# intel/rho-diffusion

Measured on AMD Instinct MI355X. Metric: denoising_steps_per_sec, higher is better.
Workload: dtype bf16; 1 GPU; DDPM reverse step, UNetv2 3D 64^3 mc=64 (BASELINE configs[2]), batch 32/GPU, bf16, LinearSchedule(1000,1e-3,0.02); global_batch=32, hip_graph=True

## Files before the change

### rho_diffusion_amd/csrc/conv.hip

```cpp
#include <cstdio>
#include <cstdlib>
#include <type_traits>

#include "conv_common.h"

#define RHO_GB_WIDE 3
#ifndef RHO_GB_BM32
#define RHO_GB_BM32 1
#endif

struct ConvK {
    const char* x1;
    const char* x2;
    const float* pre_a;
    const float* pre_b;
    const char* w;
    const float* bias;
    const char* res;
    const float* res_add;
    char* y;
    char* y2;
    int c1, c2, cin;
    int cout, coutp, split;
    int D, H, W;
// ... 4 lines not shown
    int tiles_h, tiles_w;
    int res_add_stride;
    int y2_cl;
    const char* res2;
    int pair_lg;
    int zs_h, zs_w;
    int Hs, Ws;
    float* stats;
    int tps;
    int lgTW, lgTH;
    float inv_ihw, inv_iw;
    int cofast;
    int coef_off;
    int pad_h, pad_w, oy_mul, oy_add, ox_mul, ox_add, Ho_out, Wo_out;
    int stats_off;
    int iy_mul, iy_add, ix_mul, ix_add;
    const char* gnb_x1;
    const char* gnb_x2;
    const float* gnb_a;
    const float* gnb_b;
    int gnb_c1, gnb_silu;
    int ksplit;
    float* slab;
    long long slab_stride;
    const char* sk_x1;
    const char* sk_x2;
    const char* sk_w;
    const float* sk_bias;
    int sk_c1, sk_c2;
    const char* gna_g;
    const float* gna_cA;
    const float* gna_cP;
    const float* gna_cQ;
};

__device__ __forceinline__ int fdiv_small(int a, float inv) { return (int)(((float)a + 0.5f) * inv); }


__device__ __forceinline__ int unit_position(int u, int k, int TW, int pair_lg) {
    if (TW == 8 && pair_lg >= 0) {
        const int lo = u & ((1 << pair_lg) - 1);
        const int row = ((u >> pair_lg) << (pair_lg + 1)) | lo | ((k >> 3) << pair_lg);
        return row * 8 + (k & 7);
    }
    return u * 16 + k;
}
__device__ __forceinline__ int tile_position(int m, int c, int TW, int pair_lg) {
    const int q = c >> 2;
    const int g = (0x96 >> q) & 1;
    const int k = ((q >> 1) << 2) | (c & 3);
    return unit_position(2 * m + g, k, TW, pair_lg);
}

__device__ __forceinline__ int m16_hb(int i) { return (0x0FF0 >> i) & 1; }
__device__ __forceinline__ int m16_k8(int i) { return m16_hb(i) ? i - 4 : (i < 4 ? i : i - 8); }
__device__ __forceinline__ int tile_position16(int m16, int i, int TW, int pair_lg) {
    return unit_position(2 * (m16 >> 1) + m16_hb(i), 2 * m16_k8(i) + (m16 & 1), TW, pair_lg);
}

template <typename T, int KD, int KH, int KW, int BM, int MAXP, int NW, bool M16 = false, bool FSK = false, bool GNA = false>
__global__ __launch_bounds__(NW * 64, (NW == 8 || (KD * KH * KW == 1 && MAXP <= 10)) ? 2 : 1) void k_conv(const ConvK p) {
    extern __shared__ __attribute__((aligned(16))) char smem[];
    constexpr int CK = ET<T>::CK;
    constexpr int PE = ET<T>::PE;
    constexpr int NT = KD * KH * KW;
    constexpr int NTHR = NW * 64;
    constexpr int RPP = NTHR / 4;
    constexpr int WCO = NW / 4;
    constexpr int MT = BM / 32 / WCO;
    constexpr int WROWS = (BM + RPP - 1) / RPP;

    char* const halo = smem;
    char* const wbuf = smem + (size_t)p.NP * PITCH;

    const int tid = threadIdx.x;
    const int lane = tid & 63;
    const int wave = tid >> 6;
    const int wpos = wave & 3;
    const int wco = wave >> 2;
    const int half = lane >> 5;
    const int piece = tid & 3;

    int bt = blockIdx.x;
    int ct = blockIdx.y;
    if (p.cofast) {
        const int L = blockIdx.x + gridDim.x * blockIdx.y;
        const int slot = L >> 3;
        ct = slot % (int)gridDim.y;
        bt = (L & 7) * ((int)gridDim.x >> 3) + slot / (int)gridDim.y;
    } else {
        const int nt = gridDim.x, per = nt >> 3;
        if (per > 0) {
            const int full = per << 3;
            if (bt < full) bt = (bt & 7) * per + (bt >> 3);
        }
    }
    const int tw_i = bt % p.tiles_w;
    const int th_i = (bt / p.tiles_w) % p.tiles_h;
    const int td_i = bt / (p.tiles_w * p.tiles_h);
    const int co0 = ct * BM;
    const bool splitk = (KD != 3) && p.ksplit > 1;
    const int n = splitk ? 0 : (int)blockIdx.z;
    const int od0 = td_i * p.TD, oh0 = th_i * p.TH, ow0 = tw_i * p.TW;
    const int gd_base = od0 - (KD / 2);
    const int gh_base = p.up_h ? (oh0 / 2 - 1) : (oh0 * p.sh - p.pad_h);
    const int gw_base = p.up_w ? (ow0 / 2 - 1) : (ow0 * p.sw - p.pad_w);

    constexpr int NSMP = (KD == 3) ? 1 : MAXP;
    int spos[MAXP];
    int ssmp[NSMP];
    {
        const int ihw = p.IH * p.IW;
#pragma unroll
        for (int i = 0; i < MAXP; ++i) {
            const int hp = (tid >> 2) + RPP * i;
            int pos = -2, smp = 0;
            if (hp < p.NP) {
                const int id = fdiv_small(hp, p.inv_ihw);
                const int r = hp - id * ihw;
                const int ih = fdiv_small(r, p.inv_iw);
                const int iw = r - ih * p.IW;
                const int gd = gd_base + id;
                int gh = gh_base + ih, gw = gw_base + iw;
                bool ok = ((unsigned)gd < (unsigned)p.D) & ((unsigned)gh < (unsigned)p.H) & ((unsigned)gw < (unsigned)p.W);
                if (p.zs_h) { ok = ok && ((gh & 1) == 0) && ((gh >> 1) < p.Hs); gh >>= 1; }
                if (p.zs_w) { ok = ok && ((gw & 1) == 0) && ((gw >> 1) < p.Ws); gw >>= 1; }
                if (ok) {
                    pos = ((n * p.D + gd) * p.Hs + (gh * p.iy_mul + p.iy_add)) * p.Ws + (gw * p.ix_mul + p.ix_add);
                    if constexpr (KD != 3) smp = (int)((long long)pos / p.S_in);
                } else {
                    pos = -1;
                }
            }
            spos[i] = pos;
            if constexpr (KD != 3) ssmp[i] = smp;
        }
    }

    int offd[2], offh[2][KH], offw[2][KW];
#pragma unroll
    for (int j = 0; j < 2; ++j) {
        const int pp = M16 ? tile_position16(2 * (wpos * 2 + j), lane & 15, p.TW, p.pair_lg)
                           : tile_position(wpos * 2 + j, lane & 31, p.TW, p.pair_lg);
        const int pw = pp & (p.TW - 1);
        const int ph = (pp >> p.lgTW) & (p.TH - 1);
        const int pd = pp >> (p.lgTW + p.lgTH);
        offd[j] = pd * p.IH * p.IW * PITCH + 16 * (M16 ? (lane >> 4) : half);
#pragma unroll
        for (int kh = 0; kh < KH; ++kh) {
            const int ih = p.up_h ? (((ph + kh - 1) >> 1) + 1) : (ph * p.sh + kh);
            offh[j][kh] = ih * p.IW * PITCH;
        }
#pragma unroll
        for (int kw = 0; kw < KW; ++kw) {
            const int iw = p.up_w ? (((pw + kw - 1) >> 1) + 1) : (pw * p.sw + kw);
            offw[j][kw] = iw * PITCH;
        }
    }
    const int a_off = M16 ? (wco * (BM / WCO) + 16 * m16_hb(lane & 15) + 2 * m16_k8(lane & 15)) * PITCH + 16 * (lane >> 4)
                          : (wco * (BM / WCO) + (lane & 31)) * PITCH + 16 * half;

    f32x16_t acc[MT][2];
#pragma unroll
    for (int mi = 0; mi < MT; ++mi)
#pragma unroll
        for (int j = 0; j < 2; ++j)
#pragma unroll
            for (int r = 0; r < 16; ++r) acc[mi][j][r] = 0.0f;

    int ck_lo = 0, nck = p.cin / CK;
    if (splitk) {
        const int nall = nck, kz = (int)blockIdx.z;
        ck_lo = (int)((long long)nall * kz / p.ksplit);
        nck = (int)((long long)nall * (kz + 1) / p.ksplit) - ck_lo;
    }
    const size_t wrow_bytes = (size_t)p.cin * sizeof(T);

    const bool w_active = (BM >= RPP) || (tid < BM * 4);
    const char* const w_src0 = p.w + (size_t)co0 * wrow_bytes + (size_t)ck_lo * 64;
    unsigned w_voff = (unsigned)(tid >> 2) * (unsigned)wrow_bytes + (unsigned)piece * 16u;
    const size_t w_tap_stride = (size_t)p.coutp * wrow_bytes;
    int w_row = tid >> 2;
    if constexpr (M16) w_row = (w_row & ~31) + 16 * m16_hb(w_row & 15) + 2 * m16_k8(w_row & 15) + ((w_row >> 4) & 1);
    const int w_dst0 = w_row * PITCH + piece * 16;
    constexpr int G = 1;
    constexpr int NS = NT / G;
    constexpr int PD = (NS % 3 == 0) ? 3 : 1;
    constexpr int SLOT = G * BM * PITCH;
    uint4 wq0[PD][G], wq1[PD][G];
#pragma unroll
    for (int i = 0; i < PD; ++i)
#pragma unroll
        for (int g = 0; g < G; ++g) wq0[i][g] = wq1[i][g] = make_uint4(0u, 0u, 0u, 0u);
#define RHO_LOAD_W(set_, ck_, st_)                                                                       \
    do {                                                                                                \
        _Pragma("unroll") for (int g_ = 0; g_ < G; ++g_) {                                              \
            const char* ws_ = w_src0 + (size_t)((st_) * G + g_) * w_tap_stride + (size_t)(ck_) * 64;    \
            if (w_active) wq0[set_][g_] = *reinterpret_cast<const uint4*>(ws_ + w_voff);                \
            if constexpr (WROWS == 2) wq1[set_][g_] = *reinterpret_cast<const uint4*>(ws_ + RPP * wrow_bytes + w_voff); \
        }                                                                                               \
    } while (0)
#define RHO_LOAD_WP(set_, st_)                                                                          \
    do {                                                                                                \
        if (w_active) wq0[set_][0] = *reinterpret_cast<const uint4*>(wl + w_voff);                      \
        if constexpr (WROWS == 2) wq1[set_][0] = *reinterpret_cast<const uint4*>(wl + RPP * wrow_bytes + w_voff); \
        if (((st_) + LD) % NS == NS - 1) wl = w_src0 + (size_t)min(ck + ((st_) + LD) / NS + 1, nck - 1) * 64; \
        else wl += w_tap_stride;                                                                        \
    } while (0)
#define RHO_STORE_W(buf_, set_)                                                                         \
    do {                                                                                                \
        _Pragma("unroll") for (int g_ = 0; g_ < G; ++g_) {                                              \
            char* wd_ = wbuf + (size_t)(buf_) * SLOT + g_ * BM * PITCH + w_dst0;                        \
            if (w_active) *reinterpret_cast<uint4*>(wd_) = wq0[set_][g_];                               \
            if constexpr (WROWS == 2) *reinterpret_cast<uint4*>(wd_ + RPP * PITCH) = wq1[set_][g_];     \
        }                                                                                               \
    } while (0)

    constexpr bool PIPE = (NS % 3 == 0) && (G == 1);
    constexpr int GB = (NS % 9 == 0 && ((BM == 128 && NW == 8 && M16) || (RHO_GB_BM32 && BM == 32 && !M16))) ? RHO_GB_WIDE : 1;
    constexpr int RS = (GB == 3) ? 9 : 3;
    constexpr int DS = GB + 1;
    constexpr int LD = DS + 2;
    const float* coef = nullptr;
    if constexpr (NT != 1 && KD == 3) {
        if (p.coef_off > 0 && p.pre_a != nullptr) {
            float* cw_ = reinterpret_cast<float*>(smem + p.coef_off);
            for (int i = tid; i < p.cin; i += NTHR) {
                cw_[i] = p.pre_a[(size_t)n * p.cin + i];
                cw_[p.cin + i] = p.pre_b[(size_t)n * p.cin + i];
            }
            coef = cw_;
            __syncthreads();
        }
    }
    if constexpr (FSK) {
        static_assert(M16 && MT == 2 && KD == 3, "folded skip: the 64-couts-per-wave 16x16x32 layout of the 3-D kernels");
        typedef float f32x4_t __attribute__((ext_vector_type(4)));
        typedef unsigned int u32x4_t __attribute__((ext_vector_type(4)));
        constexpr int XR = 256 / RPP;
        const int skc = p.sk_c1 + p.sk_c2, nsk = skc / CK;
        char* const sa = smem;
        char* const sw = smem + 2 * 256 * PITCH;
        int gp[XR];
#pragma unroll
        for (int i = 0; i < XR; ++i) {
            const int r = (tid >> 2) + RPP * i;
            const int od = od0 + (r >> (p.lgTW + p.lgTH)), oh = oh0 + ((r >> p.lgTW) & (p.TH - 1)), ow = ow0 + (r & (p.TW - 1));
            const bool ok = od < p.Do && oh < p.Ho && ow < p.Wo;
            gp[i] = ok ? ((n * p.Do + od) * p.Ho + oh) * p.Wo + ow : -1;
        }
        int cb[2];
#pragma unroll
        for (int j = 0; j < 2; ++j)
            cb[j] = tile_position16(2 * (wpos * 2 + j), lane & 15, p.TW, p.pair_lg) * PITCH + 16 * (lane >> 4);
        const unsigned skw_voff = (unsigned)(tid >> 2) * (unsigned)skc * (unsigned)sizeof(T) + (unsigned)piece * 16u;
        const char* const skw0 = p.sk_w + (size_t)co0 * skc * sizeof(T);
        uint4 xr[XR], wr0 = make_uint4(0u, 0u, 0u, 0u), wr1 = make_uint4(0u, 0u, 0u, 0u);
        auto sk_load = [&](int c) {
            const int ch = c * CK;
            const char* src;
            int cs, csrc;
            if (ch < p.sk_c1) { src = p.sk_x1; cs = p.sk_c1; csrc = ch; } else { src = p.sk_x2; cs = p.sk_c2; csrc = ch - p.sk_c1; }
#pragma unroll
            for (int i = 0; i < XR; ++i) {
                const int ps = gp[i] > 0 ? gp[i] : 0;
                xr[i] = *reinterpret_cast<const uint4*>(src + ((size_t)ps * cs + csrc) * sizeof(T) + piece * 16);
            }
            const char* ws_ = skw0 + (size_t)c * 64;
            if (w_active) wr0 = *reinterpret_cast<const uint4*>(ws_ + skw_voff);
            if constexpr (WROWS == 2) wr1 = *reinterpret_cast<const uint4*>(ws_ + (size_t)RPP * skc * sizeof(T) + skw_voff);
        };
        auto sk_store = [&](int slot) {
// ... 423 lines not shown
            RHO_ONE_TAIL(0, I0, std::true_type)
            if constexpr (DX == 4) {
                RHO_ONE_TAIL(1, I1, std::true_type)
                RHO_ONE_TAIL(2, I2, std::true_type)
            }
        } else {
            int ck0 = 0;
            for (; ck0 + DX <= nck; ck0 += DX) {
                RHO_ONE_STEP(0, I0, std::false_type)
                RHO_ONE_STEP(1, I1, std::false_type)
                if constexpr (DX == 4) {
                    RHO_ONE_STEP(2, I2, std::false_type)
                    RHO_ONE_STEP(3, I3, std::false_type)
                }
            }
            RHO_ONE_TAIL(0, I0, std::false_type)
            if constexpr (DX == 4) {
                RHO_ONE_TAIL(1, I1, std::false_type)
                RHO_ONE_TAIL(2, I2, std::false_type)
            }
        }
#undef RHO_ONE_STEP
#undef RHO_ONE_TAIL
    }
#undef RHO_PHASE
#undef RHO_FENCE
#undef RHO_LOAD_W
#undef RHO_LOAD_WP
#undef RHO_STORE_W
#undef RHO_HALO_LOAD
    const __attribute__((address_space(4))) ConvK* qp = (const __attribute__((address_space(4))) ConvK*)__builtin_amdgcn_kernarg_segment_ptr();
    asm volatile("" : "+s"(qp));
    const __attribute__((address_space(4))) ConvK& q = *qp;
    if (splitk) {
        float* const slab = q.slab + (size_t)blockIdx.z * q.slab_stride;
#pragma unroll
        for (int jx = 0; jx < (M16 ? 4 : 2); ++jx) {
            const int pp = M16 ? tile_position16(wpos * 4 + jx, lane & 15, q.TW, q.pair_lg) : tile_position(wpos * 2 + jx, lane & 31, q.TW, q.pair_lg);
            const int pw = pp & (q.TW - 1);
            const int ph = (pp >> q.lgTW) & (q.TH - 1);
            const int pd = pp >> (q.lgTW + q.lgTH);
            const int od = od0 + pd, oh = oh0 + ph, ow = ow0 + pw;
            if (od >= q.Do || oh >= q.Ho || ow >= q.Wo) continue;
            const size_t L = ((size_t)od * q.Ho + oh) * q.Wo + ow;
            const int j = M16 ? (jx >> 1) : jx;
#pragma unroll
            for (int mi = 0; mi < MT; ++mi) {
#pragma unroll
                for (int rx = 0; rx < (M16 ? 2 : 4); ++rx) {
                    const int rg = M16 ? 2 * rx + (jx & 1) : rx;
                    const int co = M16 ? co0 + wco * (BM / WCO) + 16 * (2 * mi + rx) + 4 * (lane >> 4)
                                       : co0 + wco * (BM / WCO) + mi * 32 + rg * 8 + half * 4;
                    *reinterpret_cast<float4*>(slab + L * q.coutp + co) =
                        make_float4(acc[mi][j][rg * 4 + 0], acc[mi][j][rg * 4 + 1], acc[mi][j][rg * 4 + 2], acc[mi][j][rg * 4 + 3]);
                }
            }
        }
        return;
    }
    const bool reg2 = q.y2_cl && co0 >= q.split && ((q.cout - q.split) % PE == 0);
    const bool cl_region = (co0 < q.split) || reg2;
    if (cl_region) {
        const int rw = reg2 ? q.cout - q.split : q.split;
        const int rc0 = reg2 ? co0 - q.split : co0;
        char* const ry = reg2 ? q.y2 : q.y;
        const char* const rrp = reg2 ? q.res2 : q.res;
        const float* const radd = reg2 ? nullptr : q.res_add;
        constexpr int ROWB = BM * 4 + 16;
        constexpr int PPR = BM / PE;
        static_assert(NTHR % PPR == 0, "a thread keeps one channel piece across its rows (statistics accumulators)");
        char* const stg = smem;
        float ssum[PE], ssq[PE];
#pragma unroll
        for (int e = 0; e < PE; ++e) ssum[e] = ssq[e] = 0.0f;
        {
            __syncthreads();
            {
#pragma unroll
                for (int j = 0; j < 2; ++j) {
#pragma unroll
                    for (int mi = 0; mi < MT; ++mi)
#pragma unroll
                        for (int rg = 0; rg < 4; ++rg) {
                            const int lr = M16 ? wpos * 64 + (2 * j + (rg & 1)) * 16 + (lane & 15) : wpos * 64 + j * 32 + (lane & 31);
                            const int cl = M16 ? wco * (BM / WCO) + 16 * (2 * mi + (rg >> 1)) + 4 * (lane >> 4)
                                               : wco * (BM / WCO) + mi * 32 + rg * 8 + half * 4;
                            *reinterpret_cast<float4*>(stg + lr * ROWB + cl * 4) =
                                make_float4(acc[mi][j][rg * 4 + 0], acc[mi][j][rg * 4 + 1], acc[mi][j][rg * 4 + 2], acc[mi][j][rg * 4 + 3]);
                        }
                }
            }
            constexpr int NIT = 256 * PPR / NTHR;
            static_assert(256 * PPR % NTHR == 0, "whole items per thread");
            int eoff[NIT];
            uint4 rres[GNA ? 1 : NIT];
            uint4 gx[NIT];
            float bia[PE];
            float gna[PE], gnb[PE];
            const bool gnb_on = q.gnb_x1 != nullptr;
            const bool gna_on = GNA && q.gna_g != nullptr;
            uint4 gg[GNA ? NIT : 1];
            float gca[GNA ? PE : 1], gcp[GNA ? PE : 1], gcq[GNA ? PE : 1];
            {
                const int piece = tid % PPR;
                const int gco = co0 + piece * PE;
                const bool g_first = gco < q.gnb_c1;
                const char* const gsrc = g_first ? q.gnb_x1 : q.gnb_x2;
                const int gC = gna_on ? q.cout : q.split;
                const int gcs = g_first ? q.gnb_c1 : gC - q.gnb_c1, gch = g_first ? gco : gco - q.gnb_c1;
                if (gnb_on) {
                    const int nsg = n + bt / q.tps;
#pragma unroll
                    for (int e = 0; e < PE; ++e) {
                        gna[e] = q.gnb_a[(size_t)nsg * gC + gco + e];
                        gnb[e] = q.gnb_b[(size_t)nsg * gC + gco + e];
                    }
                    if constexpr (GNA) {
                        const int cpg = gC / 32;
#pragma unroll
                        for (int e = 0; e < PE; ++e) {
                            const int ce = (gco + e < gC) ? gco + e : gC - 1;
                            gca[e] = q.gna_cA[(size_t)nsg * gC + ce];
                            gcp[e] = q.gna_cP[(size_t)nsg * 32 + ce / cpg];
                            gcq[e] = q.gna_cQ[(size_t)nsg * 32 + ce / cpg];
                        }
                    }
                }
#pragma unroll
                for (int q4 = 0; q4 < PE / 4; ++q4) {
                    const float4 b4 = *reinterpret_cast<const float4*>(q.bias + co0 + piece * PE + q4 * 4);
                    bia[q4 * 4 + 0] = b4.x; bia[q4 * 4 + 1] = b4.y; bia[q4 * 4 + 2] = b4.z; bia[q4 * 4 + 3] = b4.w;
                    if constexpr (FSK) {
                        if (q.sk_bias != nullptr) {
                            const float4 s4 = *reinterpret_cast<const float4*>(q.sk_bias + co0 + piece * PE + q4 * 4);
                            bia[q4 * 4 + 0] += s4.x; bia[q4 * 4 + 1] += s4.y; bia[q4 * 4 + 2] += s4.z; bia[q4 * 4 + 3] += s4.w;
                        }
                    }
                    if constexpr (KD == 3) {
                        if (radd != nullptr) {
                            const float4 e = *reinterpret_cast<const float4*>(radd + (long long)n * q.res_add_stride + co0 + piece * PE + q4 * 4);
                            bia[q4 * 4 + 0] += e.x; bia[q4 * 4 + 1] += e.y; bia[q4 * 4 + 2] += e.z; bia[q4 * 4 + 3] += e.w;
                        }
                    }
                }
#pragma unroll
                for (int k = 0; k < NIT; ++k) {
                    const int lr = tid / PPR + k * (NTHR / PPR);
                    const int pp = M16 ? tile_position16((lr >> 6) * 4 + ((lr >> 4) & 3), lr & 15, q.TW, q.pair_lg)
                                       : tile_position((lr >> 6) * 2 + ((lr >> 5) & 1), lr & 31, q.TW, q.pair_lg);
                    const int pw = pp & (q.TW - 1);
                    const int ph = (pp >> q.lgTW) & (q.TH - 1);
                    const int pd = pp >> (q.lgTW + q.lgTH);
                    const int od = od0 + pd, oh = oh0 + ph, ow = ow0 + pw;
                    const bool ok = od < q.Do && oh < q.Ho && ow < q.Wo && (rc0 + piece * PE + PE <= rw);
                    const int L = ((n * q.Do + od) * q.Ho_out + (oh * q.oy_mul + q.oy_add)) * q.Wo_out + (ow * q.ox_mul + q.ox_add);
                    eoff[k] = ok ? L : -1;
                    if constexpr (!GNA) {
                        rres[k] = make_uint4(0u, 0u, 0u, 0u);
                        if (ok && rrp != nullptr)
                            rres[k] = *reinterpret_cast<const uint4*>(rrp + ((size_t)(unsigned)L * (unsigned)rw + (unsigned)(rc0 + piece * PE)) * sizeof(T));
                    }
                    gx[k] = make_uint4(0u, 0u, 0u, 0u);
                    if (ok && gnb_on) gx[k] = *reinterpret_cast<const uint4*>(gsrc + ((size_t)(unsigned)L * (unsigned)gcs + (unsigned)gch) * sizeof(T));
                    if constexpr (GNA) {
                        gg[k] = make_uint4(0u, 0u, 0u, 0u);
                        if (ok) gg[k] = *reinterpret_cast<const uint4*>(q.gna_g + ((size_t)(unsigned)L * (unsigned)gC + (unsigned)gco) * sizeof(T));
                    }
                }
            }
            __syncthreads();
#pragma unroll
            for (int k = 0; k < NIT; ++k) {
                if (eoff[k] < 0) continue;
                const int lr = tid / PPR + k * (NTHR / PPR), piece = tid % PPR;
                const int L = eoff[k];
                const int co = co0 + piece * PE;
                float v[PE];
#pragma unroll
                for (int q4 = 0; q4 < PE / 4; ++q4) {
                    const float4 a4 = *reinterpret_cast<const float4*>(stg + lr * ROWB + (piece * PE + q4 * 4) * 4);
                    v[q4 * 4 + 0] = a4.x + bia[q4 * 4 + 0]; v[q4 * 4 + 1] = a4.y + bia[q4 * 4 + 1];
                    v[q4 * 4 + 2] = a4.z + bia[q4 * 4 + 2]; v[q4 * 4 + 3] = a4.w + bia[q4 * 4 + 3];
                }
                if (KD != 3 && radd != nullptr) {
                    const long long ns = (long long)L / q.S_out;
#pragma unroll
                    for (int q4 = 0; q4 < PE / 4; ++q4) {
                        const float4 e = *reinterpret_cast<const float4*>(radd + ns * q.res_add_stride + co + q4 * 4);
                        v[q4 * 4 + 0] += e.x; v[q4 * 4 + 1] += e.y; v[q4 * 4 + 2] += e.z; v[q4 * 4 + 3] += e.w;
// ... 69 lines not shown
                            float dz = v[e];
                            if (q.gnb_silu) dz *= dsilu_f(fmaf(gna[e], xv[e], gnb[e]));
                            ssum[e] += dz;
                            ssq[e] = fmaf(dz, xv[e], ssq[e]);
                        }
                    } else {
#pragma unroll
                        for (int e = 0; e < PE; ++e) {
                            ssum[e] += v[e];
                            ssq[e] = fmaf(v[e], v[e], ssq[e]);
                        }
                    }
                }
            }
        }
        if (q.stats != nullptr) {
            __syncthreads();
            float* red = reinterpret_cast<float*>(stg);
#pragma unroll
            for (int e = 0; e < PE; ++e) {
                red[tid * (2 * PE) + e] = ssum[e];
                red[tid * (2 * PE) + PE + e] = ssq[e];
            }
            __syncthreads();
            const int ns = n + bt / q.tps, ts = bt % q.tps + q.stats_off;
            for (int item = tid; item < PPR * 2 * PE; item += NTHR) {
                const int piece = item / (2 * PE), e2 = item % (2 * PE);
                float accv = 0.0f;
                for (int q = 0; q < NTHR / PPR; ++q) accv += red[(q * PPR + piece) * (2 * PE) + e2];
                const int stat = e2 / PE, ch = co0 + piece * PE + (e2 % PE);
                q.stats[(((size_t)ns * q.tps + ts) * 2 + stat) * q.split + ch] = accv;
            }
        }
        return;
    }
#pragma unroll
    for (int jx = 0; jx < (M16 ? 4 : 2); ++jx) {
        const int pp = M16 ? tile_position16(wpos * 4 + jx, lane & 15, q.TW, q.pair_lg) : tile_position(wpos * 2 + jx, lane & 31, q.TW, q.pair_lg);
        const int pw = pp & (q.TW - 1);
        const int ph = (pp >> q.lgTW) & (q.TH - 1);
        const int pd = pp >> (q.lgTW + q.lgTH);
        const int od = od0 + pd, oh = oh0 + ph, ow = ow0 + pw;
        if (od >= q.Do || oh >= q.Ho || ow >= q.Wo) continue;
        const long long L = (((long long)n * q.Do + od) * q.Ho + oh) * q.Wo + ow;
        const long long ns = L / q.S_out;
        const long long ps = L - ns * q.S_out;
        const int j = M16 ? (jx >> 1) : jx;
#pragma unroll
        for (int mi = 0; mi < MT; ++mi) {
#pragma unroll
            for (int rx = 0; rx < (M16 ? 2 : 4); ++rx) {
                const int rg = M16 ? 2 * rx + (jx & 1) : rx;
                const int co = M16 ? co0 + wco * (BM / WCO) + 16 * (2 * mi + rx) + 4 * (lane >> 4)
                                   : co0 + wco * (BM / WCO) + mi * 32 + rg * 8 + half * 4;
                const float4 bv = *reinterpret_cast<const float4*>(q.bias + co);
                float v0 = acc[mi][j][rg * 4 + 0] + bv.x;
                float v1 = acc[mi][j][rg * 4 + 1] + bv.y;
                float v2 = acc[mi][j][rg * 4 + 2] + bv.z;
                float v3 = acc[mi][j][rg * 4 + 3] + bv.w;
                if (cl_region) {
                    if (q.res_add != nullptr) {
                        const float4 e = *reinterpret_cast<const float4*>(q.res_add + ns * q.res_add_stride + co);
                        v0 += e.x; v1 += e.y; v2 += e.z; v3 += e.w;
                    }
                    const size_t eo = (size_t)L * q.split + co;
                    if constexpr (sizeof(T) == 2) {
                        if (q.res != nullptr) {
                            const uint2 r = *reinterpret_cast<const uint2*>(q.res + eo * 2);
// ... 12 lines not shown
                    const int w2 = q.cout - q.split;
                    const size_t eo = (size_t)L * w2 + (co - q.split);
                    if (co < q.cout) {
                        if constexpr (sizeof(T) == 2) {
                            if (q.res2 != nullptr) {
                                const uint2 r = *reinterpret_cast<const uint2*>(q.res2 + eo * 2);
                                v0 += __uint_as_float(r.x << 16); v1 += __uint_as_float(r.x & 0xFFFF0000u);
                                v2 += __uint_as_float(r.y << 16); v3 += __uint_as_float(r.y & 0xFFFF0000u);
                            }
                            *reinterpret_cast<uint2*>(q.y2 + eo * 2) = make_uint2(pack_bf16x2(v0, v1), pack_bf16x2(v2, v3));
                        } else {
                            if (q.res2 != nullptr) {
                                const float4 r = *reinterpret_cast<const float4*>(q.res2 + eo * 4);
                                v0 += r.x; v1 += r.y; v2 += r.z; v3 += r.w;
                            }
                            *reinterpret_cast<float4*>(q.y2 + eo * 4) = make_float4(v0, v1, v2, v3);
                        }
                    }
                } else {
                    const float vv[4] = {v0, v1, v2, v3};
#pragma unroll
                    for (int e = 0; e < 4; ++e) {
                        if (co + e < q.cout) {
                            const size_t eo = ((size_t)ns * (q.cout - q.split) + (co + e - q.split)) * q.S_out + ps;
                            if (q.y2_f32 || sizeof(T) == 4)
                                reinterpret_cast<float*>(q.y2)[eo] = vv[e];
                            else
                                reinterpret_cast<bf16_raw*>(q.y2)[eo] = f32_to_bf16(vv[e]);
                        }
                    }
                }
            }
        }
    }
}

struct SplitMap {
    int Ho, Wo, Ho_out, Wo_out, oy_mul, oy_add, ox_mul, ox_add;
};
struct SplitOut {
    int cout, coutp, split;
    const float* bias;
    const float* res_add;
    long long res_add_stride, S_out;
    const char* res;
    char* y;
    const char* res2;
    char* y2;
};
template <typename T>
__global__ __launch_bounds__(256) void k_splitk_reduce(const float* __restrict__ slab, long long slab_stride, int ksplit, long long positions,
                                                       SplitOut o, SplitMap m) {
    const int c4 = o.coutp / 4;
    const long long item = (long long)blockIdx.x * 256 + threadIdx.x;
    if (item >= positions * c4) return;
    const long long Ls = item / c4;
    int co = (int)(item - Ls * c4) * 4;
    if (co >= o.cout) return;
    const size_t so = (size_t)Ls * o.coutp + co;
    float4 a = *reinterpret_cast<const float4*>(slab + so);
    for (int s = 1; s < ksplit; ++s) {
        const float4 b = *reinterpret_cast<const float4*>(slab + (size_t)s * slab_stride + so);
        a.x += b.x; a.y += b.y; a.z += b.z; a.w += b.w;
    }
    long long L = Ls;
    if (m.oy_mul != 1 || m.ox_mul != 1) {
// ... 92 lines not shown
#define RHO_CASE(bm)                                                                   \
    if (BM == bm) {                                                                    \
        if (np <= 640) return launch_one<T, KD, KH, KW, bm, 10, 4>(k, grid, lds, st);  \
        if constexpr (!PHASE) return launch_one<T, KD, KH, KW, bm, 28, 4>(k, grid, lds, st); \
    }
    RHO_CASE(32)
    RHO_CASE(64)
#undef RHO_CASE
    return RHO_E_ARG;
}

template <typename T>
int launch_taps(const rho_conv_desc& d, const ConvK& k, int BM, int np, dim3 grid, size_t lds, bool m16, hipStream_t st) {
    if (d.kd == 3 && d.kh == 3 && d.kw == 3) return launch_bm<T, 3, 3, 3>(k, BM, np, grid, lds, m16, st);
    if (d.kd == 1 && d.kh == 3 && d.kw == 3) return launch_bm<T, 1, 3, 3>(k, BM, np, grid, lds, m16, st);
    if (d.kd == 1 && d.kh == 1 && d.kw == 3) return launch_bm<T, 1, 1, 3>(k, BM, np, grid, lds, m16, st);
    if (d.kd == 1 && d.kh == 1 && d.kw == 1) return launch_bm<T, 1, 1, 1>(k, BM, np, grid, lds, m16, st);
    if (d.kd == 3 && d.kh == 2 && d.kw == 2) return launch_bm<T, 3, 2, 2>(k, BM, np, grid, lds, m16, st);
    if (d.kd == 1 && d.kh == 2 && d.kw == 2) return launch_bm<T, 1, 2, 2>(k, BM, np, grid, lds, m16, st);
    if (d.kd == 1 && d.kh == 1 && d.kw == 2) return launch_bm<T, 1, 1, 2>(k, BM, np, grid, lds, m16, st);
    if (d.kd == 3 && d.kh == 1 && d.kw == 1) return launch_bm<T, 3, 1, 1>(k, BM, np, grid, lds, m16, st);
    if (d.kd == 3 && d.kh == 1 && d.kw == 2) return launch_bm<T, 3, 1, 2>(k, BM, np, grid, lds, m16, st);
    if (d.kd == 3 && d.kh == 2 && d.kw == 1) return launch_bm<T, 3, 2, 1>(k, BM, np, grid, lds, m16, st);
    return RHO_E_ARG;
}

}

static bool m16_env_on() {
    static const bool on = !(getenv("RHO_CONV_M16") && atoi(getenv("RHO_CONV_M16")) == 0);
    return on;
}

static int conv_impl(const rho_conv_desc* dp, void* stream, int64_t* stats_tiles, int64_t* ws_want = nullptr) {
    if (!dp) return RHO_E_ARG;
    const rho_conv_desc& d = *dp;
    if (!d.x1 || !d.w || !d.bias) return RHO_E_ARG;
    if (d.dtype != RHO_F32 && d.dtype != RHO_BF16) return RHO_E_ARG;
    const int CK = d.dtype == RHO_BF16 ? 32 : 16;
    const int c2 = d.x2 ? d.c2 : 0;
    const int cin = d.c1 + c2;
    if (d.c1 <= 0 || d.c1 % CK || c2 % CK) return RHO_E_ALIGN;
    if (d.cout <= 0 || d.coutp < d.cout || d.coutp % 32 || d.split < 0 || d.split > d.cout || d.split % 32) return RHO_E_ARG;
    if (d.split > 0 && !d.y) return RHO_E_ARG;
    if (d.split < d.cout && !d.y2) return RHO_E_ARG;
    if (d.split < d.cout && d.split > 0 && d.coutp != d.cout && !d.y2_cl) return RHO_E_ARG;
    if (d.y2_cl && ((d.cout - d.split) % 4 != 0)) return RHO_E_ALIGN;
    if ((d.zs_h || d.zs_w) && (d.up_h || d.up_w || d.sh != 1 || d.sw != 1 || d.out_h <= 0 || d.out_w <= 0)) return RHO_E_ARG;
    if (d.split == d.cout && d.coutp != d.cout) return RHO_E_ARG;
    if ((d.sh != 1 && d.sh != 2) || (d.sw != 1 && d.sw != 2)) return RHO_E_ARG;
    if ((d.up_h && d.sh != 1) || (d.up_w && d.sw != 1)) return RHO_E_ARG;
    if ((d.up_h && d.kh != 3) || (d.up_w && d.kw != 3)) return RHO_E_ARG;
    if (d.n <= 0 || d.d <= 0 || d.h <= 0 || d.w_ <= 0) return RHO_E_ARG;
    if (d.ph_h < 0 || d.ph_h > 2 || d.ph_w < 0 || d.ph_w > 2) return RHO_E_ARG;
    if ((d.ph_h && ((d.kh != 2 && d.kh != 1) || d.sh != 1 || d.up_h || d.zs_h)) || (d.ph_w && ((d.kw != 2 && d.kw != 1) || d.sw != 1 || d.up_w || d.zs_w)))
        return RHO_E_ARG;
    if ((!d.ph_h && !d.phd_h && d.kh == 2) || (!d.ph_w && !d.phd_w && d.kw == 2)) return RHO_E_ARG;
    if ((d.ph_h || d.ph_w) && (d.split != d.cout || d.kd == 2)) return RHO_E_ARG;
    if (d.phd_h < 0 || d.phd_h > 2 || d.phd_w < 0 || d.phd_w > 2) return RHO_E_ARG;
    if ((d.phd_h && ((d.kh != 2 && d.kh != 1) || d.sh != 1 || d.up_h || d.zs_h || d.ph_h)) ||
        (d.phd_w && ((d.kw != 2 && d.kw != 1) || d.sw != 1 || d.up_w || d.zs_w || d.ph_w)))
        return RHO_E_ARG;
    if ((d.ph_h || d.phd_h || d.ph_w || d.phd_w) && d.kd * d.kh * d.kw == 1) return RHO_E_ARG;
    if ((d.phd_h || d.phd_w) && (d.kd == 2 || d.pre_a)) return RHO_E_ARG;

    if (conv32_applies(d)) {
        if (stats_tiles) { *stats_tiles = conv32_wps(d); return 0; }
        if (ws_want) { *ws_want = 0; return 0; }
        if (g_variant != nullptr) { snprintf(g_variant->buf, (size_t)g_variant->cap, "k_conv32<bf16>"); return 0; }
        if (d.stats && d.split != d.cout) return RHO_E_ARG;
        return launch_conv32(d, as_stream(stream));
    }

    const int hv = d.zs_h ? d.out_h : d.h, wv = d.zs_w ? d.out_w : d.w_;
    const int ho = (d.ph_h || d.phd_h) ? d.h : d.up_h ? d.h * 2 : (hv + 2 * (d.kh / 2) - d.kh) / d.sh + 1;
    const int wo = (d.ph_w || d.phd_w) ? d.w_ : d.up_w ? d.w_ * 2 : (wv + 2 * (d.kw / 2) - d.kw) / d.sw + 1;
    const int ho_out = d.ph_h ? 2 * ho : ho, wo_out = d.ph_w ? 2 * wo : wo;
    const int n_phase = (d.ph_h ? 2 : 1) * (d.ph_w ? 2 : 1);
    const int phase_idx = (d.ph_h ? d.ph_h - 1 : 0) * (d.ph_w ? 2 : 1) + (d.ph_w ? d.ph_w - 1 : 0);
    const int dout = d.d;

    ConvK k{};
    int gridz = d.n;
    k.pad_h = d.kh == 1 ? 0 : d.ph_h ? 2 - d.ph_h : d.phd_h ? d.phd_h - 1 : d.kh / 2;
    k.pad_w = d.kw == 1 ? 0 : d.ph_w ? 2 - d.ph_w : d.phd_w ? d.phd_w - 1 : d.kw / 2;
    k.iy_mul = d.phd_h ? 2 : 1; k.iy_add = d.phd_h ? d.phd_h - 1 : 0;
    k.ix_mul = d.phd_w ? 2 : 1; k.ix_add = d.phd_w ? d.phd_w - 1 : 0;
    k.oy_mul = d.ph_h ? 2 : 1; k.oy_add = d.ph_h ? d.ph_h - 1 : 0;
    k.ox_mul = d.ph_w ? 2 : 1; k.ox_add = d.ph_w ? d.ph_w - 1 : 0;
    if (d.kd == 1 && d.kh == 1 && d.kw == 1) {
        if (d.sh != 1 || d.sw != 1 || d.up_h || d.up_w) return RHO_E_ARG;
        k.D = 1; k.H = 1; k.W = d.n * d.d * d.h * d.w_;
        k.Do = 1; k.Ho = 1; k.Wo = k.W;
        gridz = 1;
    } else if (d.kd == 1) {
        k.D = d.n * d.d; k.H = hv; k.W = wv;
        k.Do = k.D; k.Ho = ho; k.Wo = wo;
        gridz = 1;
    } else {
        k.D = d.d; k.H = hv; k.W = wv;
        k.Do = dout; k.Ho = ho; k.Wo = wo;
// ... 103 lines not shown
        k.gna_g = (const char*)d.gna_g; k.gna_cA = d.gna_cA; k.gna_cP = d.gna_cP; k.gna_cQ = d.gna_cQ;
        k.tps = (int)tps_geo;
    } else if (d.gnb_x1) {
        if (!d.stats || !d.gnb_a || !d.gnb_b || d.gnb_c1 <= 0 || d.gnb_c1 > d.split || d.gnb_c1 % 32 || (d.split - d.gnb_c1) % 32 ||
            ((d.gnb_c1 < d.split) != (d.gnb_x2 != nullptr)))
            return RHO_E_ARG;
        k.gnb_x1 = (const char*)d.gnb_x1; k.gnb_x2 = (const char*)d.gnb_x2; k.gnb_a = d.gnb_a; k.gnb_b = d.gnb_b;
        k.gnb_c1 = d.gnb_c1; k.gnb_silu = d.gnb_silu;
    }
    size_t lds = (size_t)t.NP * PITCH + (size_t)WSLOTS * BM * PITCH;
    k.sk_w = nullptr;
    size_t lds_sk = 0;
    if (d.sk_w) {
        if (!d.sk_x1 || d.sk_c1 <= 0 || d.sk_c1 % CK || d.sk_c2 < 0 || d.sk_c2 % CK || ((d.sk_c2 > 0) != (d.sk_x2 != nullptr))) return RHO_E_ARG;
        if (!(m16 && m16_env_on() && d.kd == 3 && d.kh == 3 && d.kw == 3 && t.NP <= 640 && (BM == 64 || BM == 128) && d.split == d.cout &&
              !d.zs_h && !d.zs_w && !d.ph_h && !d.ph_w && !d.phd_h && !d.phd_w))
            return RHO_E_ARG;
        k.sk_x1 = (const char*)d.sk_x1; k.sk_x2 = (const char*)d.sk_x2; k.sk_w = (const char*)d.sk_w; k.sk_bias = d.sk_bias;
        k.sk_c1 = d.sk_c1; k.sk_c2 = d.sk_c2;
        lds_sk = (size_t)2 * 256 * PITCH + (size_t)2 * BM * PITCH;
    }
    k.coef_off = 0;
    if (taps > 1 && d.kd == 3 && d.pre_a && lds + (size_t)2 * cin * sizeof(float) <= (BM == 128 ? lds_cap : lds_cap / 2)) {
        k.coef_off = (int)lds;
        lds += (size_t)2 * cin * sizeof(float);
    }
    if (taps == 1)
        lds = (size_t)2 * 256 * PITCH + (size_t)2 * BM * PITCH + (d.pre_a ? (size_t)2 * k.cin * sizeof(float) : 0);
    if (k.coef_off > 0 && (size_t)k.coef_off < lds_sk) { lds -= (size_t)2 * cin * sizeof(float); k.coef_off = 0; }
    if (lds < lds_sk) lds = lds_sk;
    if (d.stats) { const size_t lr = (size_t)(BM == 128 ? 512 : 256) * 16 * sizeof(float); if (lds < lr) lds = lr; }
    const size_t lds_epi = (size_t)256 * (BM * 4 + 16);
    if ((d.split > 0 || d.y2_cl) && lds < lds_epi) lds = lds_epi;
    hipStream_t st = as_stream(stream);
    const bool m16_env = m16_env_on();
    const int rc = d.dtype == RHO_BF16 ? launch_taps<bf16_raw>(d, k, BM, t.NP, grid, lds, m16 && m16_env, st)
                                       : launch_taps<float>(d, k, BM, t.NP, grid, lds, false, st);
    if (rc != 0 || ksplit == 1 || g_variant != nullptr) return rc;
    const long long items = positions * (d.coutp / 4);
    const dim3 rgrid((unsigned)((items + 255) / 256));
    const SplitMap sm{k.Ho, k.Wo, k.Ho_out, k.Wo_out, k.oy_mul, k.oy_add, k.ox_mul, k.ox_add};
    const SplitOut so{d.cout, d.coutp, d.split, d.bias, d.res_add, (long long)k.res_add_stride, k.S_out, (const char*)d.res, (char*)d.y,
                      (const char*)d.res2, (char*)d.y2};
    if (d.dtype == RHO_BF16) hipLaunchKernelGGL(k_splitk_reduce<bf16_raw>, rgrid, dim3(256), 0, st, k.slab, k.slab_stride, ksplit, positions, so, sm);
    else hipLaunchKernelGGL(k_splitk_reduce<float>, rgrid, dim3(256), 0, st, k.slab, k.slab_stride, ksplit, positions, so, sm);
    const hipError_t e = hipGetLastError();
    return e == hipSuccess ? 0 : (int)e;
}

extern "C" int64_t rho_conv_workspace_bytes(const rho_conv_desc* dp) {
    int64_t b = 0;
    return conv_impl(dp, nullptr, nullptr, &b) == 0 ? b : 0;
}

extern "C" int rho_conv_nd_fwd(const rho_conv_desc* dp, void* stream) { return conv_impl(dp, stream, nullptr); }

extern "C" int rho_conv_variant(const rho_conv_desc* dp, char* buf, int cap) {
    if (!buf || cap < 64) return RHO_E_ARG;
    buf[0] = 0;
    VariantOut vo{buf, cap};
    g_variant = &vo;
    const int rc = conv_impl(dp, nullptr, nullptr);
    g_variant = nullptr;
    return rc;
}

extern "C" int64_t rho_conv_stats_tiles(const rho_conv_desc* dp) {
    int64_t t = 0;
    return conv_impl(dp, nullptr, &t) == 0 ? t : 0;
}
```

### rho_diffusion_amd/engine/unet_engine.py

```python
from __future__ import annotations

import ctypes as C
import os
from typing import Callable, Dict, List, Optional, Tuple

import torch
from torch import nn

from .. import hip
from ..hip import check, ptr
from . import ops
from .backward_plan import BackwardBuilder

Tensor = torch.Tensor


class _ConvW:

    def __init__(self, weight: nn.Parameter, bias: nn.Parameter, dtype, row_src: Optional[Tensor] = None):
        self.weight, self.bias_param, self.dtype = weight, bias, dtype
        self.cout, self.cin = weight.shape[0], weight.shape[1]
        k = list(weight.shape[2:])
        while len(k) < 3:
            k.insert(0, 1)
# ... 370 lines not shown
                              space=torch.cat(vals).to(dev).contiguous(),
                              key_off=torch.tensor(off, dtype=torch.int32, device=dev),
                              tables=torch.tensor(list(sig), dtype=torch.int64, device=dev))
        return self._cond_dev

    def param_order(self) -> List[nn.Parameter]:
        emb = list(self.model.time_embed.parameters())
        for blk in self._film_blocks:
            emb.extend(blk.emb_layers[1].parameters())
        if getattr(self.model, "cond_fn", None) is not None:
            emb.extend(self.model.cond_fn.parameters())
        emb_ids = {id(p_) for p_ in emb}
        main = [p_ for p_ in self.model.parameters() if id(p_) not in emb_ids]
        return emb + main

    def forward(self, x: Tensor, timesteps: Tensor, y: Optional[Tensor] = None,
                t_scalar_dev: Optional[Tensor] = None, train: bool = False) -> Tensor:
        hip.require_gpu(x, "x")
        if x.dtype != torch.float32:
            x = x.float()
        x = x.contiguous()
        self.refresh_weights()
        key = (tuple(x.shape), y is not None, bool(train)) + self._plan_signature()
        plan = self._plans.get(key)
        if plan is None:
            with torch.inference_mode(False), torch.no_grad():
                plan = self._plans[key] = _Plan(self, tuple(x.shape), y is not None, bool(train))
        if train:
            self._last_train_plan = plan
        return plan.run(x, timesteps, y, t_scalar_dev)

    _PLAN_ENV = ("RHO_TRAIN_MATERIALIZE", "RHO_MATERIALIZE_MIN_COUT", "RHO_PHASE_UPSAMPLE", "RHO_PHASE_UPSAMPLE_BWD", "RHO_PHASE_MIN_WGS",
                 "RHO_FOLD_SKIP", "RHO_S2_SPLIT", "RHO_S2_SPLIT_BWD", "RHO_FUSE_GN_BWD", "RHO_GEMM_ENDS", "RHO_DIRECT_ENDS",
                 "RHO_FUSE_SKIP_DGRAD")

    def _plan_signature(self) -> tuple:
        ck = tuple(bool(b.use_checkpoint) for b in self._film_blocks)
        env = tuple(os.environ.get(k) for k in self._PLAN_ENV)
        drop = bool(self.model.training) if any(float(getattr(b, "dropout", 0.0) or 0.0) > 0.0 for b in self._film_blocks) else None
        return (ck, ops.deterministic(), env, drop)

    def drop_plans(self, train_only: bool = False) -> None:
        self._plans = {k: v for k, v in self._plans.items() if train_only and not k[2]}
        self._last_train_plan = None

    def backward(self, dpred: Tensor, on_ready: Optional[Callable[[List[nn.Parameter]], None]] = None) -> None:
        plan = self._last_train_plan
        if plan is None:
            raise hip.RhoHipError("backward() without a preceding forward(train=True)")
        with torch.no_grad():
            plan.run_backward(dpred, on_ready)


class _Plan:

    def __init__(self, eng: UNetEngine, xshape: Tuple[int, ...], has_y: bool, train: bool):
        from ..models.unet_v2 import AttentionBlock, Downsample, ResBlock, Upsample
        self.eng = eng
        self.train = train
        self.materialize_act = os.environ.get("RHO_TRAIN_MATERIALIZE", "1") != "0"
        self.materialize_min_cout = int(os.environ.get("RHO_MATERIALIZE_MIN_COUT", "256"))
        self.phase_upsample = os.environ.get("RHO_PHASE_UPSAMPLE", "1") != "0"
        self.phase_upsample_bwd = os.environ.get("RHO_PHASE_UPSAMPLE_BWD", "1") != "0"
        self.phase_min_wgs = int(os.environ.get("RHO_PHASE_MIN_WGS", "256"))
        self.fold_skip = eng.dtype == torch.bfloat16 and os.environ.get("RHO_FOLD_SKIP", "1") != "0"
        self.s2_split = os.environ.get("RHO_S2_SPLIT", "1") != "0"
        self.s2_split_bwd = os.environ.get("RHO_S2_SPLIT_BWD", "1") != "0"
        self.fuse_gn_bwd = int(os.environ.get("RHO_FUSE_GN_BWD", "128"))
        self.fuse_skip_dgrad = os.environ.get("RHO_FUSE_SKIP_DGRAD", "1") != "0"
        m = eng.model
        dt = eng.dtype
        dtc = hip.dtype_code(dt)
        dev = eng.device
        self.ops: List[Callable[[int], int]] = []
        self.info: List[dict] = []
        self.keep: List[object] = []
        self.tstats: Dict[int, Tuple[Tensor, int]] = {}
        self.nodes: List[dict] = []
        self.fwd_descs: List[object] = []
        self.wgrad_descs: List[tuple] = []
        self.cond_src = None
        self.drop_active = bool(eng.model.training) and any(float(getattr(b, "dropout", 0.0) or 0.0) > 0.0 for b in eng._film_blocks)
        self.drop_ctr = torch.zeros(1, dtype=torch.int64, device=eng.device) if self.drop_active else None
        self.drop_delta = 0
        self.drop_nodes: List[dict] = []
        L = hip.lib()
        self.L = L
        B = xshape[0]
        self.B = B
        self.xshape = xshape
        D, H, W = ops.spatial5(xshape[2:])
        dims = eng.dims
        e = 4 * eng.mc
        esz = 2 if dt == torch.bfloat16 else 4

        def buf(*shape, dtype=dt):
            t = torch.empty(*shape, dtype=dtype, device=dev)
            self.keep.append(t)
            return t

        scratch_of: Dict[tuple, Tensor] = {}

# ... 465 lines not shown
```

Baseline: 8.458 steps/s.

## Add batch-walk mode letting one 3x3x3 conv workgroup process several samples

Adds an optional walk mode for 3x3x3 M16 convolutions: each workgroup loops over several batch samples, reusing precomputed epilogue offsets and bias and shifting halo and output offsets per sample. Launch bounds for these kernels are raised to request two workgroups per CU. The walk length comes from RHO_CONV_WALK and defaults to 1, so the loop is normally off. The launch-bounds change does apply by default and may cause register spills.

```diff
diff --git a/rho_diffusion_amd/csrc/conv.hip b/rho_diffusion_amd/csrc/conv.hip
--- a/rho_diffusion_amd/csrc/conv.hip
+++ b/rho_diffusion_amd/csrc/conv.hip
@@ -60,6 +60,7 @@
     const float* gna_cA;
     const float* gna_cP;
     const float* gna_cQ;
+    int nbatch, nwalk;
 };
 
 __device__ __forceinline__ int fdiv_small(int a, float inv) { return (int)(((float)a + 0.5f) * inv); }
@@ -87,12 +88,13 @@
 }
 
 template <typename T, int KD, int KH, int KW, int BM, int MAXP, int NW, bool M16 = false, bool FSK = false, bool GNA = false>
-__global__ __launch_bounds__(NW * 64, (NW == 8 || (KD * KH * KW == 1 && MAXP <= 10)) ? 2 : 1) void k_conv(const ConvK p) {
+__global__ __launch_bounds__(NW * 64, (NW == 8 || (KD * KH * KW == 1 && MAXP <= 10) || (KD * KH * KW == 27 && M16)) ? 2 : 1) void k_conv(const ConvK p) {
     extern __shared__ __attribute__((aligned(16))) char smem[];
     constexpr int CK = ET<T>::CK;
     constexpr int PE = ET<T>::PE;
     constexpr int NT = KD * KH * KW;
     constexpr int NTHR = NW * 64;
+    constexpr bool WALK = (KD == 3 && KH == 3 && KW == 3 && M16);
     constexpr int RPP = NTHR / 4;
     constexpr int WCO = NW / 4;
     constexpr int MT = BM / 32 / WCO;
@@ -128,7 +130,12 @@
     const int td_i = bt / (p.tiles_w * p.tiles_h);
     const int co0 = ct * BM;
     const bool splitk = (KD != 3) && p.ksplit > 1;
-    const int n = splitk ? 0 : (int)blockIdx.z;
+    int n = splitk ? 0 : (int)blockIdx.z;
+    int nwk = 1;
+    if constexpr (WALK) {
+        n = (int)blockIdx.z * p.nwalk;
+        nwk = min(p.nwalk, p.nbatch - n);
+    }
     const int od0 = td_i * p.TD, oh0 = th_i * p.TH, ow0 = tw_i * p.TW;
     const int gd_base = od0 - (KD / 2);
     const int gh_base = p.up_h ? (oh0 / 2 - 1) : (oh0 * p.sh - p.pad_h);
@@ -189,12 +196,6 @@
                           : (wco * (BM / WCO) + (lane & 31)) * PITCH + 16 * half;
 
     f32x16_t acc[MT][2];
-#pragma unroll
-    for (int mi = 0; mi < MT; ++mi)
-#pragma unroll
-        for (int j = 0; j < 2; ++j)
-#pragma unroll
-            for (int r = 0; r < 16; ++r) acc[mi][j][r] = 0.0f;
 
     int ck_lo = 0, nck = p.cin / CK;
     if (splitk) {
@@ -249,6 +250,59 @@
     constexpr int RS = (GB == 3) ? 9 : 3;
     constexpr int DS = GB + 1;
     constexpr int LD = DS + 2;
+    constexpr int ROWB = BM * 4 + 16;
+    constexpr int PPR = BM / PE;
+    constexpr int NIT = 256 * PPR / NTHR;
+    static_assert(NTHR % PPR == 0, "a thread keeps one channel piece across its rows (statistics accumulators)");
+    static_assert(256 * PPR % NTHR == 0, "whole items per thread");
+    int eoff_w[WALK ? NIT : 1];
+    float bia_w[WALK ? PE : 1];
+    (void)eoff_w; (void)bia_w;
+    if constexpr (WALK) {
+#pragma unroll
+        for (int k = 0; k < NIT; ++k) eoff_w[k] = -1;
+#pragma unroll
+        for (int e = 0; e < PE; ++e) bia_w[e] = 0.0f;
+        const bool reg2 = p.y2_cl && co0 >= p.split && ((p.cout - p.split) % PE == 0);
+        if ((co0 < p.split) || reg2) {
+            const int rw = reg2 ? p.cout - p.split : p.split;
+            const int rc0 = reg2 ? co0 - p.split : co0;
+            const int piece = tid % PPR;
+#pragma unroll
+            for (int q4 = 0; q4 < PE / 4; ++q4) {
+                const float4 b4 = *reinterpret_cast<const float4*>(p.bias + co0 + piece * PE + q4 * 4);
+                bia_w[q4 * 4 + 0] = b4.x; bia_w[q4 * 4 + 1] = b4.y; bia_w[q4 * 4 + 2] = b4.z; bia_w[q4 * 4 + 3] = b4.w;
+                if constexpr (FSK) {
+                    if (p.sk_bias != nullptr) {
+                        const float4 s4 = *reinterpret_cast<const float4*>(p.sk_bias + co0 + piece * PE + q4 * 4);
+                        bia_w[q4 * 4 + 0] += s4.x; bia_w[q4 * 4 + 1] += s4.y; bia_w[q4 * 4 + 2] += s4.z; bia_w[q4 * 4 + 3] += s4.w;
+                    }
+                }
+            }
+#pragma unroll
+            for (int k = 0; k < NIT; ++k) {
+                const int lr = tid / PPR + k * (NTHR / PPR);
+                const int pp = M16 ? tile_position16((lr >> 6) * 4 + ((lr >> 4) & 3), lr & 15, p.TW, p.pair_lg)
+                                   : tile_position((lr >> 6) * 2 + ((lr >> 5) & 1), lr & 31, p.TW, p.pair_lg);
+                const int pw = pp & (p.TW - 1);
+                const int ph = (pp >> p.lgTW) & (p.TH - 1);
+                const int pd = pp >> (p.lgTW + p.lgTH);
+                const int od = od0 + pd, oh = oh0 + ph, ow = ow0 + pw;
+                const bool ok = od < p.Do && oh < p.Ho && ow < p.Wo && (rc0 + piece * PE + PE <= rw);
+                const int L = ((n * p.Do + od) * p.Ho_out + (oh * p.oy_mul + p.oy_add)) * p.Wo_out + (ow * p.ox_mul + p.ox_add);
+                eoff_w[k] = ok ? L : -1;
+            }
+        }
+    }
+
+#pragma unroll 1
+    for (int wi = 0; wi < nwk; ++wi) {
+#pragma unroll
+    for (int mi = 0; mi < MT; ++mi)
+#pragma unroll
+        for (int j = 0; j < 2; ++j)
+#pragma unroll
+            for (int r = 0; r < 16; ++r) acc[mi][j][r] = 0.0f;
     const float* coef = nullptr;
     if constexpr (NT != 1 && KD == 3) {
         if (p.coef_off > 0 && p.pre_a != nullptr) {
@@ -266,6 +320,9 @@
         typedef float f32x4_t __attribute__((ext_vector_type(4)));
         typedef unsigned int u32x4_t __attribute__((ext_vector_type(4)));
         constexpr int XR = 256 / RPP;
+        int tid_f = tid;
+        asm volatile("" : "+v"(tid_f));
+        const int tid = tid_f, lane = tid & 63, wpos = (tid >> 6) & 3, piece = tid & 3;
         const int skc = p.sk_c1 + p.sk_c2, nsk = skc / CK;
         char* const sa = smem;
         char* const sw = smem + 2 * 256 * PITCH;
@@ -755,6 +812,11 @@
     const __attribute__((address_space(4))) ConvK* qp = (const __attribute__((address_space(4))) ConvK*)__builtin_amdgcn_kernarg_segment_ptr();
     asm volatile("" : "+s"(qp));
     const __attribute__((address_space(4))) ConvK& q = *qp;
+    int tid_e = tid;
+    if constexpr (WALK) asm volatile("" : "+v"(tid_e));
+    {
+    const int tid = tid_e, lane = tid & 63, wave = tid >> 6, wpos = wave & 3, wco = wave >> 2, half = lane >> 5;
+    (void)wco; (void)half;
     if (splitk) {
         float* const slab = q.slab + (size_t)blockIdx.z * q.slab_stride;
 #pragma unroll
@@ -779,8 +841,7 @@
                 }
             }
         }
-        return;
-    }
+    } else {
     const bool reg2 = q.y2_cl && co0 >= q.split && ((q.cout - q.split) % PE == 0);
     const bool cl_region = (co0 < q.split) || reg2;
     if (cl_region) {
@@ -789,9 +850,6 @@
         char* const ry = reg2 ? q.y2 : q.y;
         const char* const rrp = reg2 ? q.res2 : q.res;
         const float* const radd = reg2 ? nullptr : q.res_add;
-        constexpr int ROWB = BM * 4 + 16;
-        constexpr int PPR = BM / PE;
-        static_assert(NTHR % PPR == 0, "a thread keeps one channel piece across its rows (statistics accumulators)");
         char* const stg = smem;
         float ssum[PE], ssq[PE];
 #pragma unroll
@@ -813,8 +871,6 @@
                         }
                 }
             }
-            constexpr int NIT = 256 * PPR / NTHR;
-            static_assert(256 * PPR % NTHR == 0, "whole items per thread");
             int eoff[NIT];
             uint4 rres[GNA ? 1 : NIT];
             uint4 gx[NIT];
@@ -851,13 +907,12 @@
                 }
 #pragma unroll
                 for (int q4 = 0; q4 < PE / 4; ++q4) {
-                    const float4 b4 = *reinterpret_cast<const float4*>(q.bias + co0 + piece * PE + q4 * 4);
-                    bia[q4 * 4 + 0] = b4.x; bia[q4 * 4 + 1] = b4.y; bia[q4 * 4 + 2] = b4.z; bia[q4 * 4 + 3] = b4.w;
-                    if constexpr (FSK) {
-                        if (q.sk_bias != nullptr) {
-                            const float4 s4 = *reinterpret_cast<const float4*>(q.sk_bias + co0 + piece * PE + q4 * 4);
-                            bia[q4 * 4 + 0] += s4.x; bia[q4 * 4 + 1] += s4.y; bia[q4 * 4 + 2] += s4.z; bia[q4 * 4 + 3] += s4.w;
-                        }
+                    if constexpr (WALK) {
+                        bia[q4 * 4 + 0] = bia_w[q4 * 4 + 0]; bia[q4 * 4 + 1] = bia_w[q4 * 4 + 1];
+                        bia[q4 * 4 + 2] = bia_w[q4 * 4 + 2]; bia[q4 * 4 + 3] = bia_w[q4 * 4 + 3];
+                    } else {
+                        const float4 b4 = *reinterpret_cast<const float4*>(q.bias + co0 + piece * PE + q4 * 4);
+                        bia[q4 * 4 + 0] = b4.x; bia[q4 * 4 + 1] = b4.y; bia[q4 * 4 + 2] = b4.z; bia[q4 * 4 + 3] = b4.w;
                     }
                     if constexpr (KD == 3) {
                         if (radd != nullptr) {
@@ -868,16 +923,23 @@
                 }
 #pragma unroll
                 for (int k = 0; k < NIT; ++k) {
-                    const int lr = tid / PPR + k * (NTHR / PPR);
-                    const int pp = M16 ? tile_position16((lr >> 6) * 4 + ((lr >> 4) & 3), lr & 15, q.TW, q.pair_lg)
-                                       : tile_position((lr >> 6) * 2 + ((lr >> 5) & 1), lr & 31, q.TW, q.pair_lg);
-                    const int pw = pp & (q.TW - 1);
-                    const int ph = (pp >> q.lgTW) & (q.TH - 1);
-                    const int pd = pp >> (q.lgTW + q.lgTH);
-                    const int od = od0 + pd, oh = oh0 + ph, ow = ow0 + pw;
-                    const bool ok = od < q.Do && oh < q.Ho && ow < q.Wo && (rc0 + piece * PE + PE <= rw);
-                    const int L = ((n * q.Do + od) * q.Ho_out + (oh * q.oy_mul + q.oy_add)) * q.Wo_out + (ow * q.ox_mul + q.ox_add);
-                    eoff[k] = ok ? L : -1;
+                    if constexpr (WALK) {
+                        eoff[k] = eoff_w[k];
+                        asm volatile("" : "+v"(eoff[k]));
+                    } else {
+                        const int lr = tid / PPR + k * (NTHR / PPR);
+                        const int pp = M16 ? tile_position16((lr >> 6) * 4 + ((lr >> 4) & 3), lr & 15, q.TW, q.pair_lg)
+                                           : tile_position((lr >> 6) * 2 + ((lr >> 5) & 1), lr & 31, q.TW, q.pair_lg);
+                        const int pw = pp & (q.TW - 1);
+                        const int ph = (pp >> q.lgTW) & (q.TH - 1);
+                        const int pd = pp >> (q.lgTW + q.lgTH);
+                        const int od = od0 + pd, oh = oh0 + ph, ow = ow0 + pw;
+                        const bool ok_ = od < q.Do && oh < q.Ho && ow < q.Wo && (rc0 + piece * PE + PE <= rw);
+                        const int L_ = ((n * q.Do + od) * q.Ho_out + (oh * q.oy_mul + q.oy_add)) * q.Wo_out + (ow * q.ox_mul + q.ox_add);
+                        eoff[k] = ok_ ? L_ : -1;
+                    }
+                    const int L = eoff[k];
+                    const bool ok = L >= 0;
                     if constexpr (!GNA) {
                         rres[k] = make_uint4(0u, 0u, 0u, 0u);
                         if (ok && rrp != nullptr)
@@ -1013,8 +1075,7 @@
                 q.stats[(((size_t)ns * q.tps + ts) * 2 + stat) * q.split + ch] = accv;
             }
         }
-        return;
-    }
+    } else {
 #pragma unroll
     for (int jx = 0; jx < (M16 ? 4 : 2); ++jx) {
         const int pp = M16 ? tile_position16(wpos * 4 + jx, lane & 15, q.TW, q.pair_lg) : tile_position(wpos * 2 + jx, lane & 31, q.TW, q.pair_lg);
@@ -1093,6 +1154,21 @@
                 }
             }
         }
+    }
+    }
+    }
+    }
+    if constexpr (WALK) {
+        if (wi + 1 < nwk) {
+            __syncthreads();
+            ++n;
+            const int s_in = (int)q.S_in, s_out = (int)q.S_out;
+#pragma unroll
+            for (int i = 0; i < MAXP; ++i) spos[i] += spos[i] >= 0 ? s_in : 0;
+#pragma unroll
+            for (int k = 0; k < NIT; ++k) eoff_w[k] += eoff_w[k] >= 0 ? s_out : 0;
+        }
+    }
     }
 }
 
@@ -1251,7 +1327,21 @@
     return on;
 }
 
-static int conv_impl(const rho_conv_desc* dp, void* stream, int64_t* stats_tiles, int64_t* ws_want = nullptr) {
+static int conv_walk_length(const rho_conv_desc& d, bool m16_variant, int np, long long wgs_per_sample) {
+    const bool legal = m16_variant && d.kd == 3 && d.kh == 3 && d.kw == 3 && d.n >= 2 && d.sh == 1 && d.sw == 1 && !d.up_h && !d.up_w && !d.zs_h && !d.zs_w &&
+                       !d.ph_h && !d.ph_w && !d.phd_h && !d.phd_w && !d.gnb_x1 && !d.gna_g && d.split == d.cout && np <= 640;
+    if (!legal) return 1;
+    const char* const e = getenv("RHO_CONV_WALK");
+    if (e != nullptr && *e != 0) {
+        const int v = atoi(e);
+        if (v == 0 || v == 1) return 1;
+        if (v == 2 || v == 4 || v == 8) return v;
+    }
+    (void)wgs_per_sample;
+    return 1;
+}
+
+static int conv_impl(const rho_conv_desc* dp, void* stream, int64_t* stats_tiles, int64_t* ws_want = nullptr, int* walk_out = nullptr) {
     if (!dp) return RHO_E_ARG;
     const rho_conv_desc& d = *dp;
     if (!d.x1 || !d.w || !d.bias) return RHO_E_ARG;
@@ -1286,6 +1376,7 @@
     if (conv32_applies(d)) {
         if (stats_tiles) { *stats_tiles = conv32_wps(d); return 0; }
         if (ws_want) { *ws_want = 0; return 0; }
+        if (walk_out) { *walk_out = 1; return 0; }
         if (g_variant != nullptr) { snprintf(g_variant->buf, (size_t)g_variant->cap, "k_conv32<bf16>"); return 0; }
         if (d.stats && d.split != d.cout) return RHO_E_ARG;
         return launch_conv32(d, as_stream(stream));
@@ -1455,6 +1546,12 @@
     if (d.stats) { const size_t lr = (size_t)(BM == 128 ? 512 : 256) * 16 * sizeof(float); if (lds < lr) lds = lr; }
     const size_t lds_epi = (size_t)256 * (BM * 4 + 16);
     if ((d.split > 0 || d.y2_cl) && lds < lds_epi) lds = lds_epi;
+    k.nbatch = d.n; k.nwalk = 1;
+    if (d.kd == 3) {
+        k.nwalk = conv_walk_length(d, m16 && m16_env_on() && BM >= 64, t.NP, tiles * (d.coutp / BM));
+        grid.z = (unsigned)cdiv(d.n, k.nwalk);
+    }
+    if (walk_out) { *walk_out = k.nwalk; return 0; }
     hipStream_t st = as_stream(stream);
     const bool m16_env = m16_env_on();
     const int rc = d.dtype == RHO_BF16 ? launch_taps<bf16_raw>(d, k, BM, t.NP, grid, lds, m16 && m16_env, st)
@@ -1488,6 +1585,11 @@
     return rc;
 }
 
+extern "C" int rho_conv_walk_length(const rho_conv_desc* dp) {
+    int w = 0;
+    return conv_impl(dp, nullptr, nullptr, nullptr, &w) == 0 ? w : 0;
+}
+
 extern "C" int64_t rho_conv_stats_tiles(const rho_conv_desc* dp) {
     int64_t t = 0;
     return conv_impl(dp, nullptr, &t) == 0 ? t : 0;
diff --git a/rho_diffusion_amd/engine/unet_engine.py b/rho_diffusion_amd/engine/unet_engine.py
--- a/rho_diffusion_amd/engine/unet_engine.py
+++ b/rho_diffusion_amd/engine/unet_engine.py
@@ -426,7 +426,7 @@
 
     _PLAN_ENV = ("RHO_TRAIN_MATERIALIZE", "RHO_MATERIALIZE_MIN_COUT", "RHO_PHASE_UPSAMPLE", "RHO_PHASE_UPSAMPLE_BWD", "RHO_PHASE_MIN_WGS",
                  "RHO_FOLD_SKIP", "RHO_S2_SPLIT", "RHO_S2_SPLIT_BWD", "RHO_FUSE_GN_BWD", "RHO_GEMM_ENDS", "RHO_DIRECT_ENDS",
-                 "RHO_FUSE_SKIP_DGRAD")
+                 "RHO_FUSE_SKIP_DGRAD", "RHO_CONV_WALK")
 
     def _plan_signature(self) -> tuple:
         ck = tuple(bool(b.use_checkpoint) for b in self._film_blocks)
@@ -462,6 +462,7 @@
         self.s2_split_bwd = os.environ.get("RHO_S2_SPLIT_BWD", "1") != "0"
         self.fuse_gn_bwd = int(os.environ.get("RHO_FUSE_GN_BWD", "128"))
         self.fuse_skip_dgrad = os.environ.get("RHO_FUSE_SKIP_DGRAD", "1") != "0"
+        self.conv_walk = os.environ.get("RHO_CONV_WALK")
         m = eng.model
         dt = eng.dtype
         dtc = hip.dtype_code(dt)
```

Result: slower. 8.373 steps/s (-1.0%).
